# zhuhaozh/metadrive_ped

Hardware: AMD Instinct MI355X
Metric: agent-steps/sec at 4096 envs x 240-beam lidar (higher is better)
Workload: dtype f32; 1 GPU; BASELINE configs[1]: 4096 batched MetaDriveEnv per GPU, 3-block PG map (reference default block distribution: curves, straights, ramps, X/T intersections, roundabouts), 240-beam lidar, traffic_density=0.1, trigger traffic, auto-reset; envs_per_gpu=4096, agents_per_env=1, mover_capacity=24, n_beams=240

## Files before the change

### include/md_entity.h

```cpp
#ifndef MD_ENTITY_H
#define MD_ENTITY_H

#include "md_geom.h"
#include "md_lane_change.h"

MD_HD int md_scene_of_env(const MdState* g, int e) { return g->scene_of ? g->scene_of[e] : e; }
MD_HD size_t md_track_stride(const MdState* s, const MdConfig* c) {
    return (size_t)(s->walk.n_scenes > 0 ? s->walk.n_scenes : c->n_envs) * (size_t)c->cap;
}
MD_HD int md_scene(const MdState* s, int e) { return s->scene_of ? s->scene_of[0] : e; }

MD_HD MdState md_env_view(const MdState* g, const MdConfig* c, int e) {
    MdState v = *g;
    const size_t b = (size_t)e * (size_t)c->cap;
    const size_t bs = (size_t)md_scene_of_env(g, e) * (size_t)c->cap;
    const size_t a = (size_t)e * (size_t)c->agents_per_env;
    v.shape = g->shape + b;
    v.dyn = g->dyn ? g->dyn + b : 0;
    v.param = g->param ? g->param + b : 0;
    v.nav = g->nav ? g->nav + b : 0;
    v.pid = g->pid ? g->pid + b : 0;
    v.action = g->action ? g->action + 2 * b : 0;
    v.route_nodes = g->route_nodes ? g->route_nodes + b * MD_ROUTE_LEN : 0;
    v.route_roads = g->route_roads ? g->route_roads + b * MD_ROUTE_LEN : 0;
    v.final_lane = g->final_lane ? g->final_lane + b : 0;
    v.idm_rand = g->idm_rand ? g->idm_rand + b * MD_IDM_RAND : 0;
    v.flags = g->flags ? g->flags + b : 0;
    v.obs = g->obs ? g->obs + a * (size_t)c->obs_dim : 0;
    v.reward = g->reward ? g->reward + a : 0;
    v.cost = g->cost ? g->cost + a : 0;
    v.step_info = g->step_info ? g->step_info + a * 8 : 0;
    v.need_reset = g->need_reset ? g->need_reset + e : 0;
    v.shape0 = g->shape0 ? g->shape0 + b : 0;
    v.dyn0 = g->dyn0 ? g->dyn0 + b : 0;
    v.nav0 = g->nav0 ? g->nav0 + b : 0;
    v.pid0 = g->pid0 ? g->pid0 + b : 0;
    v.param0 = g->param0 ? g->param0 + b : 0;
    v.done_out = g->done_out ? g->done_out + 4 * a : 0;
    v.idle_ring = g->idle_ring ? g->idle_ring + a * MD_IDLE_WINDOW : 0;
    v.route_nodes0 = g->route_nodes0 ? g->route_nodes0 + b * MD_ROUTE_LEN : 0;
    v.route_roads0 = g->route_roads0 ? g->route_roads0 + b * MD_ROUTE_LEN : 0;
    v.final_lane0 = g->final_lane0 ? g->final_lane0 + b : 0;
    v.rng = g->rng ? g->rng + e : 0;
    v.env_steps = g->env_steps ? g->env_steps + e : 0;
    v.agent_id = g->agent_id ? g->agent_id + b : 0;
    v.next_agent_id = g->next_agent_id ? g->next_agent_id + e : 0;
    v.detected = g->detected ? g->detected + (size_t)e * c->agents_per_env * 2 : 0;
    v.agent_action = g->agent_action ? g->agent_action + (size_t)e * c->agents_per_env * 2 : 0;
    v.track_shape = g->track_shape ? g->track_shape + bs : 0;
    v.track_dyn = g->track_dyn ? g->track_dyn + 2 * bs : 0;
    v.scene_of = g->scene_of ? g->scene_of + e : 0;
    v.walk_ep = g->walk_ep ? g->walk_ep + e : 0;
    v.route_n = g->route_n ? g->route_n + 4 * b : 0;
    v.route_segs = g->route_segs ? g->route_segs + b * (size_t)c->route_seg_cap : 0;
    v.route_verts = g->route_verts ? g->route_verts + 2 * b * (size_t)c->route_vert_cap : 0;
    v.route_aux = g->route_aux ? g->route_aux + 8 * b : 0;
    return v;
}

MD_HD int md_obs_base(const MdConfig* c) { return c->random_agent_model ? 2 : 0; }
MD_HD int md_obs_mid(const MdConfig* c) { return md_obs_base(c) + (c->n_side > 0 ? c->n_side : 2); }
MD_HD int md_obs_ll(const MdConfig* c) { return md_obs_mid(c) + 6; }
MD_HD int md_obs_navi(const MdConfig* c) { return md_obs_ll(c) + (c->n_lane_line > 0 ? c->n_lane_line : 1); }
MD_HD int md_is_tollgate(const MdConfig* c) { return c->is_multi_agent && c->ma_kind == MD_MA_TOLLGATE; }
MD_HD int md_navi_dims(const MdConfig* c) { return md_is_tollgate(c) ? 0 : 10; }
MD_HD int md_obs_tail(const MdConfig* c) { return md_is_tollgate(c) ? 2 : 0; }
MD_HD int md_obs_others(const MdConfig* c) { return md_obs_navi(c) + md_navi_dims(c); }
MD_HD int md_others_width(const MdConfig* c) { return c->add_others_navi ? 8 : 4; }
MD_HD int md_obs_lidar(const MdConfig* c) { return md_obs_others(c) + (c->num_others > 0 ? c->num_others * md_others_width(c) : 0); }

MD_HD uint32_t md_done_word(uint32_t fl) {
    return ((fl & MD_FL_TERMINATED) ? 1u : 0u) | ((fl & MD_FL_TRUNCATED) ? 0x100u : 0u) | ((fl & 0xFFFFu) << 16);
}
MD_HD int md_kind_of(int flags) { return flags & MD_KIND_MASK; }
MD_HD int md_is_circle_kind(int k) { return k == MD_KIND_CONE || k == MD_KIND_WARNING || k == MD_KIND_PEDESTRIAN; }
MD_HD int md_present(int flags) { return (flags & MD_F_ALIVE) && md_kind_of(flags) != MD_KIND_NONE; }
MD_HD int md_drives(int flags) {
    return md_present(flags) && md_kind_of(flags) == MD_KIND_VEHICLE && !(flags & (MD_F_STATIC | MD_F_PENDING));
}

MD_HD int md_walks(int flags) {
    const int k = md_kind_of(flags);
    return (flags & MD_F_ALIVE) && !(flags & MD_F_STATIC) && (k == MD_KIND_PEDESTRIAN || k == MD_KIND_CYCLIST);
}
// ... 55 lines not shown
    float thr = md_sanitize(s->action[2 * n + 1]);
    s->action[2 * n] = steer;
    s->action[2 * n + 1] = thr;
    float yaw = (sh->s * d->last_c - sh->c * d->last_s) / (float)c->substeps;
    d->last_x = sh->cx;
    d->last_y = sh->cy;
    d->last_c = sh->c;
    d->last_s = sh->s;
    d->steering = steer;
    d->throttle = thr;
    float x = sh->cx, y = sh->cy, psi = d->heading, v = d->speed;
    MdBicycle bike;
    md_bicycle_prepare(steer, thr, v, sh->hl, sh->hw, c->dt, c->enable_reverse && (sh->flags & MD_F_AGENT), &s->param[n], &bike);
    float c0, s0;
    md_sincos(psi, &s0, &c0);
    float cp = c0 * bike.cb - s0 * bike.sb, sp = s0 * bike.cb + c0 * bike.sb;
    for (int k = 0; k < c->substeps; ++k) md_bicycle_substep(&x, &y, &psi, &v, &cp, &sp, &yaw, thr, &bike, &s->param[n], c->dt);
    sh->cx = x;
    sh->cy = y;
    d->heading = psi;
    d->speed = v;
    md_sincos(psi, &sh->s, &sh->c);
}


#define MD_OBS_TASKS 9

typedef struct MdObsCtx {
    const MdLane *lane, *ref0, *ref_last, *next0, *fin, *rl;
    float cur_w, cur_n, positive_road;
    int valid;
    int cur_block;
} MdObsCtx;

MD_HD void md_observe_ctx(const MdLane* lanes, const MdRoad* roads, const MdState* s, int n, MdObsCtx* k) {
    const MdShape* sh = &s->shape[n];
    const MdNav* nav = &s->nav[n];
    k->valid = md_drives(sh->flags) && nav->lane >= 0;
    k->lane = k->ref0 = k->ref_last = k->next0 = k->fin = k->rl = lanes;
    k->cur_w = k->cur_n = k->positive_road = 0.0f;
    k->cur_block = 0;
    if (!k->valid) return;
    const MdRoad* cur_road = &roads[nav->road0];
    k->cur_block = cur_road->block_kind;
    int has_next = nav->ck1 != nav->ck0;
    const MdRoad* next_road = has_next ? &roads[nav->road1] : cur_road;
    k->lane = &lanes[nav->lane];
    k->ref0 = &lanes[cur_road->first_lane];
    k->ref_last = &lanes[cur_road->first_lane + cur_road->n_lanes - 1];
    k->next0 = &lanes[next_road->first_lane];
    k->fin = &lanes[s->final_lane[n]];
    k->cur_w = k->lane->width;
    k->cur_n = (float)cur_road->n_lanes;
    k->positive_road = 1.0f;
    if (k->lane->road == nav->road0) k->rl = k->lane;
    else {
        k->rl = k->ref0;
        k->positive_road = cur_road->negative ? -1.0f : 1.0f;
    }
}

MD_HD void md_observe_task(int task, const MdObsCtx* k, const MdState* s, const MdConfig* c, int n, float* out5) {
    const MdShape* sh = &s->shape[n];
    const MdDyn* d = &s->dyn[n];
    float x = sh->cx, y = sh->cy;
    out5[0] = out5[1] = out5[2] = out5[3] = out5[4] = 0.0f;
    if (!k->valid) return;
    if (task == 0 || task == 2 || task == 5 || task == 6 || task == 7) {
        const MdLane* L = (task == 0) ? k->ref0 : ((task == 2) ? k->lane : ((task == 5) ? k->fin : k->rl));
        float px = (task == 6) ? d->last_x : x;
        float py = (task == 6) ? d->last_y : y;
        md_lane_local(L, px, py, &out5[0], &out5[1]);
    } else if (task == 3 || task == 4) {
        md_navi_for_checkpoint((task == 3) ? k->ref0 : k->next0, (k->cur_n / 2.0f - 0.5f) * k->cur_w, x, y, sh->c, sh->s,
                               k->cur_n, k->cur_w, c->curve_radius_max, c->curve_angle_max, out5);
    } else if (task == 1) {
        out5[0] = md_heading_diff(k->ref_last, x, y, sh->c, sh->s);
    } else if (task == 8) {
        float cosb = (sh->c * d->last_c + sh->s * d->last_s) / (md_norm(sh->c, sh->s) * md_norm(d->last_c, d->last_s));
        float beta = md_acos(md_clip(cosb, 0.0f, 1.0f));
        out5[0] = md_clip(beta / 0.1f, 0.0f, 1.0f);
        out5[1] = md_step_energy(md_fabs(d->speed) * 3.6f, md_norm(d->last_x - x, d->last_y - y));
    }
}

MD_HD void md_route_borders(const MdObsCtx* k, const float (*r)[5], float* to_left, float* to_right) {
    *to_left = r[0][1] + k->cur_w / 2.0f;
    *to_right = k->cur_w * k->cur_n - *to_left;
}

MD_HD void md_observe_state_dims(const MdObsCtx* k, const MdState* s, const MdConfig* c, int n, const float (*r)[5], float* obs) {
    const MdDyn* d = &s->dyn[n];
    const int o_mid = md_obs_mid(c), o_ll = md_obs_ll(c), o_navi = md_obs_navi(c);
    float to_left, to_right;
    md_route_borders(k, r, &to_left, &to_right);
    float speed_kmh = md_fabs(d->speed) * 3.6f;
    const MdParam* P = &s->param[n];
    const int o_base = md_obs_base(c);
    if (o_base) {
        obs[0] = md_clip(2.0f * s->shape[n].hl / 10.0f, 0.0f, 1.0f);
        obs[1] = md_clip(2.0f * s->shape[n].hw / 2.5f, 0.0f, 1.0f);
    }
    if (c->n_side <= 0) {
        obs[o_base + 0] = md_clip(to_left / c->total_width, 0.0f, 1.0f);
        obs[o_base + 1] = md_clip(to_right / c->total_width, 0.0f, 1.0f);
    }
    obs[o_mid + 0] = r[1][0];
    obs[o_mid + 1] = md_clip((speed_kmh + 1.0f) / (P->max_speed_kmh + 1.0f), 0.0f, 1.0f);
    obs[o_mid + 2] = md_clip((d->steering / 60.0f + 1.0f) / 2.0f, 0.0f, 1.0f);
    obs[o_mid + 3] = md_clip((s->action[2 * n] + 1.0f) / 2.0f, 0.0f, 1.0f);
    obs[o_mid + 4] = md_clip((s->action[2 * n + 1] + 1.0f) / 2.0f, 0.0f, 1.0f);
    obs[o_mid + 5] = r[8][0];
    float llat = r[2][1];
    if (c->n_lane_line <= 0) obs[o_ll] = md_clip((llat * 2.0f / c->max_lane_width + 1.0f) / 2.0f, 0.0f, 1.0f);
    if (!md_is_tollgate(c))
        for (int i = 0; i < 5; ++i) {
            obs[o_navi + i] = r[3][i];
            obs[o_navi + 5 + i] = r[4][i];
        }
}

MD_HD void md_observe_combine(const MdObsCtx* k, const MdState* s, const MdConfig* c, int a, int env_just_reset,
                              const float (*r)[5]) {
    int n = a;
    int just_reset = env_just_reset || ((s->shape[n].flags & MD_F_SPAWNED) != 0);
    s->shape[n].flags &= ~MD_F_SPAWNED;
    int ai = a;
    float* obs = s->obs + (size_t)ai * c->obs_dim;
    float* info = s->step_info + (size_t)ai * 8;
    MdDyn* d = &s->dyn[n];
    MdNav* nav = &s->nav[n];
    const int toll = md_is_tollgate(c);
    if (!k->valid) {
        if (s->done_out) ((uint32_t*)s->done_out)[ai] = 0u;
        for (int i = 0; i < md_obs_lidar(c); ++i) obs[i] = 0.0f;
        for (int i = c->obs_dim - md_obs_tail(c); i < c->obs_dim; ++i) obs[i] = 0.0f;
        s->reward[ai] = 0.0f;
        s->cost[ai] = 0.0f;
        for (int i = 0; i < 8; ++i) info[i] = 0.0f;
        return;
    }
    float cur_w = k->cur_w, cur_n = k->cur_n;

    float to_left, to_right;
    md_route_borders(k, r, &to_left, &to_right);
    uint32_t fl = s->flags[n] & (MD_FL_CRASH_VEHICLE | MD_FL_CRASH_OBJECT | MD_FL_CRASH_HUMAN | MD_FL_CRASH_BUILDING |
                                 MD_FL_CRASH_SIDEWALK | MD_FL_ON_WHITE_CONT | MD_FL_ON_YELLOW_CONT | MD_FL_ON_BROKEN |
                                 MD_FL_ON_CROSSWALK | MD_FL_ON_LANE);
    if (to_right < 0.0f || to_left < 0.0f) fl |= MD_FL_OUT_OF_ROUTE;

    md_observe_state_dims(k, s, c, n, r, obs);
    float speed_kmh = md_fabs(d->speed) * 3.6f;
    const MdParam* P = &s->param[n];
    float ls = r[2][0], llat = r[2][1];

    float fs = r[5][0], flat = r[5][1];
    int arrive = (k->fin->length - 5.0f < fs) && (fs < k->fin->length + 5.0f) && (cur_w / 2.0f >= flat) &&
                 (flat >= (0.5f - cur_n) * cur_w);
    int out_of_road = !(fl & MD_FL_ON_LANE);
    if (c->out_of_route_done) out_of_road = out_of_road || (fl & MD_FL_OUT_OF_ROUTE);
    else if (c->on_continuous_line_done)
        out_of_road = out_of_road || (fl & (MD_FL_ON_YELLOW_CONT | MD_FL_ON_WHITE_CONT | MD_FL_CRASH_SIDEWALK));
    if (toll) {
        out_of_road = (fl & MD_FL_CRASH_SIDEWALK) != 0;
        if (c->on_continuous_line_done) out_of_road = out_of_road || (fl & MD_FL_ON_YELLOW_CONT);
    }
// ... 767 lines not shown
```

### metadrive_ped_amd/csrc/mdstep.hip

```cpp
#include <hip/hip_runtime.h>
#include <stddef.h>
#include <stdint.h>
#include <stdio.h>
#include <stdlib.h>

#include <type_traits>

#include "md_curriculum.h"
#include "md_expert.h"
#include "md_expert_sense.h"
#include "md_ai_protect.h"
#include "md_scenario.h"
#include "md_topdown.h"
#include "md_render.h"

namespace {

constexpr int kBlock = 256;

enum Phase : int {
    PH_RESET = 1,
    PH_IDM = 2,
    PH_INTEGRATE = 4,
    PH_LOCALIZE = 8,
// ... 1307 lines not shown
template <bool kKeys>
__device__ __forceinline__ void idm_vehicle_wave(const MdWorld& w, const MdLane* lanes, const MdRoad* roads, const MdState& s,
                                 const MdConfig& c, int m, int slot, int lane_id, int* wave_list) {
    MdIdmPlan plan;
    plan.success = plan.use_ref = plan.fail = 0;
    plan.ids[0] = plan.ids[1] = plan.ids[2] = -1;
    const bool st_ = (slot == c.agents_per_env) && lane_id == 0;
    (void)st_;
    MD_FINE_STAMP(st_, 4);
    if (lane_id == 0) md_idm_plan(&w, lanes, roads, &s, &c, m, slot, &plan);
    if constexpr (!kKeys) {
        plan.success = bcast_i(plan.success, 0);
        plan.use_ref = bcast_i(plan.use_ref, 0);
        plan.fail = bcast_i(plan.fail, 0);
        plan.ids[0] = bcast_i(plan.ids[0], 0);
        plan.ids[1] = bcast_i(plan.ids[1], 0);
        plan.ids[2] = bcast_i(plan.ids[2], 0);
        MD_FINE_STAMP(st_, 5);
        FrontBack fb;
        idm_scan_wave(lanes, s, c, slot, lane_id, wave_list, plan, fb);
        MD_FINE_STAMP(st_, 6);
        if (lane_id == 0) md_idm_decide(lanes, roads, &s, slot, &plan, &fb);
    } else {
        plan.success = __builtin_amdgcn_readlane(plan.success, 0);
        plan.use_ref = __builtin_amdgcn_readlane(plan.use_ref, 0);
        plan.fail = __builtin_amdgcn_readlane(plan.fail, 0);
        plan.ids[0] = __builtin_amdgcn_readlane(plan.ids[0], 0);
        plan.ids[1] = __builtin_amdgcn_readlane(plan.ids[1], 0);
        plan.ids[2] = __builtin_amdgcn_readlane(plan.ids[2], 0);
        MD_FINE_STAMP(st_, 5);
        FrontBack fb;
        idm_scan_wave_keys(lanes, s, c, slot, lane_id, wave_list, plan, fb);
        MD_FINE_STAMP(st_, 6);
        if (lane_id == 0) {
            int front_obj;
            float front_dist;
            const float speed_kmh = md_fabs(s.dyn[slot].speed) * 3.6f;
            const int steer = md_idm_policy(lanes, roads, &s, slot, &plan, &fb, &front_obj, &front_dist);
            if (steer < 0) {
                s.action[2 * slot] = 0.0f;
                s.action[2 * slot + 1] = 0.0f;
            } else {
                const int k = (steer == plan.ids[0]) ? 0 : ((steer == plan.ids[1]) ? 1 : 2);
                const float* wf = reinterpret_cast<const float*>(wave_list);
                md_idm_act(&s, slot, speed_kmh, front_obj, front_dist, wf[kIdmLatWord + k], wf[kIdmHeadWord + k]);
            }
        }
    }
    MD_FINE_STAMP(st_, 7);
}

__device__ __forceinline__ void idm_group_wave(const MdWorld& w, const MdLane* lanes, const MdRoad* roads, const MdState& s,
                               const MdConfig& c, int m, int j0, unsigned long long mask, int lane_id, int* wave_list) {
    const int my_slot = j0 + lane_id;
    const bool mine = (mask >> lane_id) & 1ull;
    MdIdmPlan plan;
    plan.success = plan.use_ref = plan.fail = 0;
    plan.ids[0] = plan.ids[1] = plan.ids[2] = -1;
    if (mine) md_idm_plan(&w, lanes, roads, &s, &c, m, my_slot, &plan);
    FrontBack fb;
    front_back_clear(fb);
    unsigned long long todo = mask;
    while (todo) {
        const int v = __ffsll((long long)todo) - 1;
        todo &= todo - 1;
        MdIdmPlan up;
        up.success = bcast_i(plan.success, v);
        up.use_ref = bcast_i(plan.use_ref, v);
        up.fail = bcast_i(plan.fail, v);
        up.ids[0] = bcast_i(plan.ids[0], v);
        up.ids[1] = bcast_i(plan.ids[1], v);
        up.ids[2] = bcast_i(plan.ids[2], v);
        FrontBack ufb;
        idm_scan_wave(lanes, s, c, j0 + v, lane_id, wave_list, up, ufb);
        wave_lds_sync();
        if (lane_id == v) {
            plan.fail = up.fail;
            fb = ufb;
        }
    }
    if (mine) md_idm_decide(lanes, roads, &s, my_slot, &plan, &fb);
}

__device__ __forceinline__ void observe_agent_wave1(const MdLane* lanes, const MdRoad* roads, const MdState& s, const MdConfig& c, int a,
                                    int just_reset, int lane_id, float* wave_scratch ) {
    MdObsCtx k;
    MD_FINE_STAMP(a == 0 && lane_id == 0, 8);
    md_observe_ctx(lanes, roads, &s, a, &k);
    MD_FINE_STAMP(a == 0 && lane_id == 0, 9);
    if (lane_id < MD_OBS_TASKS) {
        float mine[5];
        md_observe_task(lane_id, &k, &s, &c, a, mine);
#pragma unroll
        for (int i = 0; i < 5; ++i) wave_scratch[lane_id * 5 + i] = mine[i];
    }
    wave_lds_sync();
    MD_FINE_STAMP(a == 0 && lane_id == 0, 10);
    if (lane_id == 0) md_observe_combine(&k, &s, &c, a, just_reset, (const float (*)[5])wave_scratch);
    __builtin_amdgcn_wave_barrier();
    MD_FINE_STAMP(a == 0 && lane_id == 0, 11);
}

constexpr int kObsGroups = 4;
constexpr int kObsScratch = kObsGroups * 48;

__device__ __forceinline__ void observe_agent_wave(const MdLane* lanes, const MdRoad* roads, const MdState& s, const MdConfig& c, int a_base,
                                   int just_reset, int lane_id, float* wave_scratch ) {
    const int g = lane_id >> 4, sub = lane_id & 15;
    const int a = a_base + g;
    const bool live = a < c.agents_per_env;
    float* scratch = wave_scratch + g * 48;
    MdObsCtx k;
    if (live) md_observe_ctx(lanes, roads, &s, a, &k);
    if (live && sub < MD_OBS_TASKS) {
        float mine[5];
        md_observe_task(sub, &k, &s, &c, a, mine);
#pragma unroll
        for (int i = 0; i < 5; ++i) scratch[sub * 5 + i] = mine[i];
    }
    wave_lds_sync();
    if (live && sub == 0) md_observe_combine(&k, &s, &c, a, just_reset, (const float (*)[5])scratch);
    __builtin_amdgcn_wave_barrier();
}

#ifndef MD_TRIGGER_EARLY
#define MD_TRIGGER_EARLY 1
#endif
constexpr int kNoTrigger = 0x7fffffff;
__device__ __forceinline__ void trigger_search_wave(const MdState& s, const MdConfig& c, int lane_id, int* min_order_out, int* trig_road_out) {
    const int base = 0;
    MD_FINE_STAMP(lane_id == 0, -1);
    *min_order_out = kNoTrigger;
    *trig_road_out = -1;
    int my_min = 0x7fffffff;
    for (int j = lane_id; j < c.cap; j += 64) {
        const int f = s.shape[base + j].flags;
        if ((f & MD_F_PENDING) && (f & MD_F_ALIVE)) {
            const int o = s.nav[base + j].trigger_order;
            my_min = o < my_min ? o : my_min;
        }
    }
    const int min_order = wave_min_i(my_min, my_min != 0x7fffffff, 0x7fffffff);
    if (min_order == 0x7fffffff) return;
    int my_slot = 0x7fffffff;
    for (int j = lane_id; j < c.cap; j += 64) {
        const int f = s.shape[base + j].flags;
        if ((f & MD_F_PENDING) && (f & MD_F_ALIVE) && s.nav[base + j].trigger_order == min_order)
            my_slot = j < my_slot ? j : my_slot;
    }
    const int first_slot = wave_min_i(my_slot, my_slot != 0x7fffffff, 0x7fffffff);
    *min_order_out = min_order;
    *trig_road_out = s.nav[base + first_slot].trigger_road;
    MD_FINE_STAMP(lane_id == 0, 14);
}

__device__ __forceinline__ void trigger_fire_wave(const MdLane* lanes, const MdState& s, const MdConfig& c, int lane_id, int min_order, int trig_road) {
    const int base = 0;
    if (min_order == kNoTrigger) return;
    bool fire = false;
    for (int a = lane_id; a < c.agents_per_env; a += 64) {
        if (!md_drives(s.shape[base + a].flags)) continue;
        const int al = s.nav[base + a].lane;
        if (al >= 0 && lanes[al].road == trig_road) fire = true;
    }
    if (__ballot(fire) == 0ull) return;
    for (int j = lane_id; j < c.cap; j += 64) {
        const int f = s.shape[base + j].flags;
        if ((f & MD_F_PENDING) && (f & MD_F_ALIVE) && s.nav[base + j].trigger_order == min_order)
            s.shape[base + j].flags = f & ~MD_F_PENDING;
    }
}

__device__ __forceinline__ void trigger_env(const MdLane* lanes, const MdState& s, const MdConfig& c, int lane_id) {
// ... 195 lines not shown
    s.param = img.param;
    s.final_lane = img.final_lane;
    return s;
}

struct SlotMask { unsigned long long lo, hi; };
static_assert(MD_MAX_CAP <= 128, "drive_mask: two 64-bit words per env");
__device__ __forceinline__ SlotMask drive_mask(const MdShape* shape, int cap, int lane) {
    SlotMask m = {0ull, 0ull};
    for (int j0 = 0; j0 < cap; j0 += 64) {
        const int j = j0 + lane;
        const unsigned long long mk = __ballot(j < cap && md_drives(shape[j < cap ? j : 0].flags));
        if (j0 == 0) m.lo = mk;
        else m.hi = mk;
    }
    return m;
}
__device__ __forceinline__ SlotMask agent_share(SlotMask m, int agents) {
    m.lo &= agents >= 64 ? ~0ull : ((1ull << agents) - 1ull);
    m.hi &= agents <= 64 ? 0ull : (agents >= 128 ? ~0ull : ((1ull << (agents - 64)) - 1ull));
    return m;
}
__device__ __forceinline__ int popc(SlotMask m) { return __popcll(m.lo) + __popcll(m.hi); }

#ifndef MD_ENV_BLOCK
#define MD_ENV_BLOCK 256
#endif
#ifndef MD_ENV_WAVES_EU
#define MD_ENV_WAVES_EU 7
#endif
template <class Config, class State, class Zero, class Null>
__host__ __device__ inline void lean_pins(Config& c, State& s, Zero zero, Null null) {
    zero(c.is_multi_agent);
    zero(c.traffic_mode);
    zero(c.agent_idm);
    zero(c.num_others);
    null(s.detected);
}
__host__ __device__ inline bool lean_pins_hold(const MdState& s, const MdConfig& c) {
    bool ok = true;
    lean_pins(c, s, [&ok](const int32_t& v) { ok = ok && v == 0; }, [&ok](const void* p) { ok = ok && p == nullptr; });
    return ok;
}
__host__ __device__ inline void lean_pins_fold(MdState& s, MdConfig& c) {
    lean_pins(c, s, [](int32_t& v) { v = 0; }, [](auto*& p) { p = nullptr; });
}

template <int PH, bool RESPAWN, bool MULTI>
constexpr int env_waves_per_eu() { return (PH == PH_ALL && !RESPAWN && !MULTI && MD_ENV_BLOCK >= 128) ? MD_ENV_WAVES_EU : 0; }

struct EnvLds { uint32_t shape, dyn, nav, pid, action, flags, lanes, roads, scratch, param, final_lane, det, onlane, cfl, tk, bytes; };
__host__ __device__ inline EnvLds env_lds(int cap, int agents, int n_lanes, int n_roads, int waves, bool multi, bool lidar_only) {
    EnvLds L;
    L.shape = 0;
    L.dyn = L.shape + (uint32_t)cap * sizeof(MdShape);
    L.nav = L.dyn + (uint32_t)cap * sizeof(MdDyn);
    L.pid = L.nav + (uint32_t)cap * sizeof(MdNav);
    L.action = L.pid + (uint32_t)cap * sizeof(MdPid);
    L.flags = L.action + (uint32_t)cap * 2 * sizeof(float);
    L.lanes = align_up(L.flags + (uint32_t)cap * sizeof(uint32_t), 16);
    L.roads = L.lanes + (uint32_t)n_lanes * sizeof(MdLane);
    L.scratch = L.roads + (uint32_t)n_roads * sizeof(MdRoad);
    L.param = L.scratch + (uint32_t)waves * (multi ? kObsScratch : 48) * sizeof(float);
    L.final_lane = L.param + (uint32_t)cap * sizeof(MdParam);
    L.det = L.final_lane + align_up(cap, 2) * sizeof(int32_t);
    L.onlane = L.det + (uint32_t)agents * 2 * sizeof(unsigned long long);
    L.cfl = L.onlane + (uint32_t)cap * sizeof(uint32_t);
    const uint32_t shared_words = 2 * cap > 8 ? 2 * cap : 8;
    L.tk = L.onlane + shared_words * sizeof(uint32_t);
    L.bytes = lidar_only ? L.dyn : L.tk + 3 * sizeof(int);
    return L;
}

template <int PH, bool STAGE_MAP, bool RESPAWN = false, bool MULTI = false, int BLK = MD_ENV_BLOCK>
__global__ __launch_bounds__(BLK)
__attribute__((amdgpu_waves_per_eu(env_waves_per_eu<PH, RESPAWN, MULTI>() ? env_waves_per_eu<PH, RESPAWN, MULTI>() : 1,
                                   env_waves_per_eu<PH, RESPAWN, MULTI>() ? env_waves_per_eu<PH, RESPAWN, MULTI>() : 8)))
void env_kernel(MdWorld w, MdState g, MdConfig c, float* lidar_out,
                                                  int lidar_stride, int lidar_offset) {
    constexpr int kBlock = BLK;
    constexpr int kWaves = kBlock / 64;
    constexpr bool kIdmKeys = !STAGE_MAP && !RESPAWN && !MULTI;
    constexpr bool kLocRoadFirst = PH == PH_ALL ? kIdmKeys : PH == PH_LOCALIZE_ROAD_FIRST;
    if constexpr (PH == PH_ALL && !RESPAWN && !MULTI && !STAGE_MAP) lean_pins_fold(g, c);
    if ((int)blockIdx.x >= c.n_envs) return;
#ifdef MD_STAMP
    const int e = g_env_order ? g_env_order[blockIdx.x] : (int)blockIdx.x;
#else
    const int e = blockIdx.x;
#endif
    const int tid = threadIdx.x;
    const int wave = tid >> 6, lane = tid & 63;
    const int cap = c.cap;

    const int n_stage_lanes = STAGE_MAP ? w.max_lanes : 0, n_stage_roads = STAGE_MAP ? w.max_roads : 0;
    constexpr bool kLidarOnly = (PH == PH_LIDAR);
    const EnvLds L = env_lds(cap, c.agents_per_env, n_stage_lanes, n_stage_roads, kWaves, MULTI, kLidarOnly);
    extern __shared__ __attribute__((aligned(16))) unsigned char smem[];
    MdShape* l_shape = reinterpret_cast<MdShape*>(smem + L.shape);
    MdDyn* l_dyn = reinterpret_cast<MdDyn*>(smem + L.dyn);
    MdNav* l_nav = reinterpret_cast<MdNav*>(smem + L.nav);
    MdPid* l_pid = reinterpret_cast<MdPid*>(smem + L.pid);
    float* l_action = reinterpret_cast<float*>(smem + L.action);
    uint32_t* l_flags = reinterpret_cast<uint32_t*>(smem + L.flags);
    MdLane* l_lanes = reinterpret_cast<MdLane*>(smem + L.lanes);
    MdRoad* l_roads = reinterpret_cast<MdRoad*>(smem + L.roads);
    float* l_scratch = reinterpret_cast<float*>(smem + L.scratch) + wave * (MULTI ? kObsScratch : 48);
    MdParam* l_param = reinterpret_cast<MdParam*>(smem + L.param);
    int32_t* l_final = reinterpret_cast<int32_t*>(smem + L.final_lane);
    unsigned long long* l_det = reinterpret_cast<unsigned long long*>(smem + L.det);
    const EnvImage img = {l_shape, l_dyn, l_pid, l_param, l_nav, l_action, l_flags, l_final};
    uint32_t* l_onlane = reinterpret_cast<uint32_t*>(smem + L.onlane);
    uint32_t* l_cfl = reinterpret_cast<uint32_t*>(smem + L.cfl);
    int* l_tk = reinterpret_cast<int*>(smem + L.tk);
    const bool track_det = (PH == PH_ALL) && (RESPAWN || MULTI) && g.detected != nullptr;

    const MdState gv = md_env_view(&g, &c, e);
    const int reset_flag = (PH & PH_RESET) ? gv.need_reset[0] : 0;

    MD_STAMP_AT(0);
    const bool kFusedAct = (PH == PH_ALL) && gv.agent_action != nullptr;
    const MdLane* lanes;
    const MdRoad* roads;
    if (STAGE_MAP) {
        lanes = l_lanes;
        roads = l_roads;
    } else {
        lanes = w.lanes + w.lane_off[w.env_map[e]];
        roads = w.roads + w.road_off[w.env_map[e]];
    }
    if (kLidarOnly) {
        copy16(l_shape, gv.shape, cap * (int)sizeof(MdShape), tid, kBlock);
    } else if (kBlock >= 256) {
        const int n32 = cap * 2, n64 = cap * 4;
        const uint4* g_shape = reinterpret_cast<const uint4*>(gv.shape);
        const uint4* g_dyn = reinterpret_cast<const uint4*>(gv.dyn);
        const uint4* g_pid = reinterpret_cast<const uint4*>(gv.pid);
        const uint4* g_param = reinterpret_cast<const uint4*>(gv.param);
        const uint4* g_nav = reinterpret_cast<const uint4*>(gv.nav);
        uint4 r_shape, r_dyn, r_pid, r_param, r_nav0;
        float2 r_act;
        uint32_t r_fl;
        int r_fin;
        const bool p32 = tid < n32, pc = tid < cap;
        if (p32) {
            r_shape = ld_stream(&g_shape[tid]);
            r_dyn = ld_stream(&g_dyn[tid]);
            r_pid = ld_stream(&g_pid[tid]);
            r_param = ld_stream(&g_param[tid]);
        }
        if (tid < n64) r_nav0 = ld_stream(&g_nav[tid]);
        if (pc) {
            r_act = (kFusedAct && tid < c.agents_per_env) ? reinterpret_cast<const float2*>(gv.agent_action)[tid]
                                                          : reinterpret_cast<const float2*>(gv.action)[tid];
            r_fl = gv.flags[tid];
            r_fin = gv.final_lane ? gv.final_lane[tid] : 0;
        }
        if (STAGE_MAP) {
            const int m = w.env_map[e];
            const int lo = w.lane_off[m], ro = w.road_off[m];
            copy16(l_lanes, w.lanes + lo, (w.lane_off[m + 1] - lo) * (int)sizeof(MdLane), tid, kBlock);
            copy16(l_roads, w.roads + ro, (w.road_off[m + 1] - ro) * (int)sizeof(MdRoad), tid, kBlock);
        }
        if (p32) {
            reinterpret_cast<uint4*>(l_shape)[tid] = r_shape;
            reinterpret_cast<uint4*>(l_dyn)[tid] = r_dyn;
// ... 111 lines not shown
            }
            if (RESPAWN) md_advance_mover(&s, &c, j);
            else md_integrate_mover(&s, &c, j);
        }
        if (!RESPAWN)
            for (int j = tid; j < cap; j += kBlock) md_walk_mover(&s, &c, j);
        __syncthreads();
    }
    MD_STAMP_AT(4);
    unsigned long long drv_lo = 0ull, drv_hi = 0ull;
    if (kFused) {
        const SlotMask drv = drive_mask(s.shape, cap, lane);
        drv_lo = drv.lo;
        drv_hi = drv.hi;
        const SlotMask adrv = agent_share(drv, c.agents_per_env);
        const unsigned long long adrv_lo = adrv.lo, adrv_hi = adrv.hi;
        const int nd = popc(drv), na = popc(adrv);
        if (MULTI) {
            const int npair = (nd + 1) >> 1;
            for (int guard = 0; guard < npair + na; ++guard) {
                int item = 0;
                if (lane == 0) item = atomicAdd(&l_tk[0], 1);
                item = __builtin_amdgcn_readfirstlane(item);
                if (item < 0 || item >= npair + na) break;
                if (item < na) contacts_vehicle(w, s, c, e, kth_bit(adrv_lo, adrv_hi, item), lane, l_cfl);
                else localize_pair(w, lanes, roads, s, e, kth_bit(drv_lo, drv_hi, 2 * (item - na)), kth_bit(drv_lo, drv_hi, 2 * (item - na) + 1), lane, l_onlane);
            }
        } else if (nd + na <= kWaves) {
            for (int item = wave; item < nd + na; item += kWaves) {
                if (item < nd) {
                    if (!(MD_ENV_SKIP & 4)) localize_vehicle<kLocRoadFirst>(w, lanes, roads, s, e, kth_bit(drv_lo, drv_hi, item), lane, l_onlane);
                } else if (!(MD_ENV_SKIP & 8)) contacts_vehicle(w, s, c, e, kth_bit(adrv_lo, adrv_hi, item - nd), lane, l_cfl);
            }
        } else {
            const int npair = (nd + 1) >> 1;
            for (int item = wave; item < npair + na; item += kWaves) {
                if (item < npair) {
                    if (!(MD_ENV_SKIP & 4)) localize_pair<kLocRoadFirst>(w, lanes, roads, s, e, kth_bit(drv_lo, drv_hi, 2 * item), kth_bit(drv_lo, drv_hi, 2 * item + 1), lane, l_onlane);
                } else if (!(MD_ENV_SKIP & 8))
                    contacts_vehicle(w, s, c, e, kth_bit(adrv_lo, adrv_hi, item - npair), lane, l_cfl);
            }
        }
        __syncthreads();
    } else {
        if (PH & PH_LOCALIZE) {
            for (int j = wave; j < cap; j += kWaves) localize_vehicle<kLocRoadFirst>(w, lanes, roads, s, e, j, lane);
            __syncthreads();
        }
        MD_STAMP_AT(5);
        if (PH & PH_CONTACTS) {
            for (int j = wave; j < cap; j += kWaves) contacts_vehicle(w, s, c, e, j, lane);
            __syncthreads();
        }
    }
    MD_STAMP_AT(6);
    if (PH & PH_TRAFFIC) {
        for (int j = tid; j < cap; j += kBlock) {
            const bool drove = kFused ? ((((j < 64) ? (drv_lo >> j) : (drv_hi >> (j - 64))) & 1ull) != 0ull) : false;
            if (kFused && !drove) continue;
            const int f = s.shape[j].flags;
            if (kFused)
                s.flags[j] = l_onlane[j] | ((f & MD_F_AGENT) ? l_cfl[j] : 0u);
            if (md_drives(f) && !(f & MD_F_AGENT) && !(s.flags[j] & MD_FL_ON_LANE)) {
                s.shape[j].flags = f & ~MD_F_ALIVE;
                if (kFused) l_cfl[j] = kRemovedMark;
            }
        }
        if (plan_ahead && wave == kWaves - 1) {
            if (kTriggerEarly) {
                const int* l_trig = reinterpret_cast<const int*>(smem + L.scratch) + kTrigWord;
                trigger_fire_wave(lanes, s, c, lane, __builtin_amdgcn_readfirstlane(l_trig[0]), __builtin_amdgcn_readfirstlane(l_trig[1]));
            } else trigger_env(lanes, s, c, lane);
        }
        __syncthreads();
        if (RESPAWN) {
            if (tid == 0) md_traffic_respawn_env(&w, lanes, &s, &c, w.env_map[e]);
            __syncthreads();
        }
    }
    MD_STAMP_AT(7);
    if (plan_ahead) {
        if (wave == 0) {
            if (!(MD_ENV_SKIP & 16))
                for (int a = 0; a < c.agents_per_env; ++a) observe_agent_wave1(lanes, roads, s, c, a, just_reset, lane, l_scratch);
        } else if (!(MD_ENV_SKIP & 2)) {
            int rank = 0;
            for (int j0 = 0; j0 < cap; j0 += 64) {
                const int jl = j0 + lane;
                const int fl = (jl < cap) ? s.shape[jl].flags : 0;
                unsigned long long mk = __ballot(jl < cap && md_drives(fl) && !(fl & MD_F_AGENT));
                while (mk) {
                    const int j = j0 + __ffsll((long long)mk) - 1;
                    mk &= mk - 1;
                    if (rank % (kWaves - 1) == wave - 1) idm_vehicle_wave<kIdmKeys>(w, lanes, roads, s, c, w.env_map[e], j, lane, reinterpret_cast<int*>(l_scratch));
                    ++rank;
                }
            }
        }
        MD_STAMP_AT(8);
    } else if (PH & PH_OBSERVE) {
        if (MULTI) {
            const int n_grp = (c.agents_per_env + kObsGroups - 1) / kObsGroups;
            for (int guard = 0; guard < n_grp; ++guard) {
                int gi = 0;
                if (lane == 0) gi = atomicAdd(&l_tk[1], 1);
                gi = __builtin_amdgcn_readfirstlane(gi);
                if (gi < 0 || gi >= n_grp) break;
                observe_agent_wave(lanes, roads, s, c, gi * kObsGroups, just_reset, lane, l_scratch);
            }
        } else {
            for (int a = wave; a < c.agents_per_env; a += kWaves) observe_agent_wave1(lanes, roads, s, c, a, just_reset, lane, l_scratch);
        }
        MD_STAMP_AT(8);
    }
    if ((PH & PH_LIDAR) && !(PH == PH_ALL && (MD_ENV_SKIP & 1))) {
        if (c.n_beams > 0) phase_lidar(w, s, c, e, tid, kWaves, lidar_out, lidar_stride, lidar_offset, track_det ? l_det : nullptr, PH == PH_ALL ? &l_tk[2] : nullptr);
    }

    MD_STAMP_AT(9);
    if (!kLidarOnly) {
        __syncthreads();
        MD_STAMP_AT(10);
        constexpr bool respawns = (PH & PH_TRAFFIC) && RESPAWN;
        if (kFused && !MULTI && !do_reset) {
            const bool replay = c.traffic_mode == 3;
            auto dirty = [&](int j) { return replay || md_moves(l_shape[j].flags) || l_cfl[j] == kRemovedMark; };
            for (int i = tid; i < cap * 2; i += kBlock)
                if (dirty(i >> 1)) {
                    st_stream(&reinterpret_cast<uint4*>(gv.shape)[i], reinterpret_cast<const uint4*>(l_shape)[i]);
                    st_stream(&reinterpret_cast<uint4*>(gv.dyn)[i], reinterpret_cast<const uint4*>(l_dyn)[i]);
                    st_stream(&reinterpret_cast<uint4*>(gv.pid)[i], reinterpret_cast<const uint4*>(l_pid)[i]);
                }
            for (int i = tid; i < cap * 4; i += kBlock)
                if (dirty(i >> 2)) st_stream(&reinterpret_cast<uint4*>(gv.nav)[i], reinterpret_cast<const uint4*>(l_nav)[i]);
            for (int j = tid; j < cap; j += kBlock)
                if (dirty(j)) {
                    reinterpret_cast<float2*>(gv.action)[j] = reinterpret_cast<const float2*>(l_action)[j];
                    gv.flags[j] = l_flags[j];
                    if (RESPAWN) gv.final_lane[j] = l_final[j];
                }
            if (track_det)
                for (int j = tid; j < 2 * c.agents_per_env; j += kBlock) gv.detected[j] = l_det[j];
            MD_STAMP_AT(11);
            return;
        }
        if (PH & (PH_RESET | PH_IDM | PH_INTEGRATE | PH_TRAFFIC | PH_OBSERVE | PH_LIFECYCLE)) copy16(gv.shape, l_shape, cap * (int)sizeof(MdShape), tid, kBlock);
        if (MULTI && (PH & (PH_RESET | PH_LIFECYCLE)) && c.random_agent_model && c.is_multi_agent)
            copy16(gv.param, l_param, cap * (int)sizeof(MdParam), tid, kBlock);
        if ((PH & (PH_RESET | PH_INTEGRATE | PH_LIFECYCLE)) || respawns) copy16(gv.dyn, l_dyn, cap * (int)sizeof(MdDyn), tid, kBlock);
        if ((PH & (PH_RESET | PH_IDM | PH_LOCALIZE | PH_OBSERVE | PH_LIFECYCLE)) || respawns) copy16(gv.nav, l_nav, cap * (int)sizeof(MdNav), tid, kBlock);
        if ((PH & (PH_RESET | PH_IDM | PH_OBSERVE | PH_LIFECYCLE)) || respawns || (lane_change && (PH & PH_INTEGRATE)))
            copy16(gv.pid, l_pid, cap * (int)sizeof(MdPid), tid, kBlock);
        if (((PH & (PH_RESET | PH_LIFECYCLE)) && MULTI) || ((PH & (PH_RESET | PH_TRAFFIC)) && RESPAWN)) {
            for (int j = tid; j < cap; j += kBlock) gv.final_lane[j] = l_final[j];
        }
        for (int j = tid; j < cap; j += kBlock) {
            if ((PH & (PH_RESET | PH_IDM | PH_INTEGRATE | PH_LIFECYCLE)) || respawns) {
                gv.action[2 * j] = l_action[2 * j];
                gv.action[2 * j + 1] = l_action[2 * j + 1];
            }
            if ((PH & (PH_RESET | PH_LOCALIZE | PH_CONTACTS | PH_OBSERVE | PH_LIFECYCLE)) || respawns) gv.flags[j] = l_flags[j];
        }
        if (track_det)
            for (int j = tid; j < 2 * c.agents_per_env; j += kBlock) gv.detected[j] = l_det[j];
        if (do_reset && tid == 0) gv.need_reset[0] = 0;
    }
    MD_STAMP_AT(11);
// ... 2831 lines not shown
```

Measured before the change: 58.54 million agent-steps/s.

## Compute observation tasks in lockstep across 16 lanes with branch-free selects

Replaces the per-lane divergent observation task dispatch with a single branch-free routine in which 16 wave lanes each compute one output. Lanes choose their lane pointer, field offsets and formula operands through mask-based selects, and inline reduced atan/asin polynomials replace the library calls. The aim is to remove SIMD divergence, since the different task branches (lane-local, navigation checkpoints, heading, energy) would otherwise serialize within the wave. The cost is duplicated arithmetic on every lane, plus inline asm and polynomial approximations that may differ slightly in numerics.

```diff
diff --git a/include/md_entity.h b/include/md_entity.h
--- a/include/md_entity.h
+++ b/include/md_entity.h
@@ -1,5 +1,7 @@
 #ifndef MD_ENTITY_H
 #define MD_ENTITY_H
+
+#include <stddef.h>
 
 #include "md_geom.h"
 #include "md_lane_change.h"
@@ -221,6 +223,170 @@
         out5[0] = md_clip(beta / 0.1f, 0.0f, 1.0f);
         out5[1] = md_step_energy(md_fabs(d->speed) * 3.6f, md_norm(d->last_x - x, d->last_y - y));
     }
+}
+
+#define MD_OBS_LANES 16
+#if defined(__HIP_DEVICE_COMPILE__)
+#define MD_LANE_IN(lane, mask) __extension__({ unsigned long long m_; __asm__ volatile("s_mov_b64 %0, %1" : "=s"(m_) : "i"(mask)); __builtin_amdgcn_inverse_ballot_w64(m_); })
+#else
+#define MD_LANE_IN(lane, mask) ((((mask) >> (lane)) & 1ull) != 0)
+#endif
+#define MD_LANE_F(m) ((int)(offsetof(MdLane, m) / sizeof(float)))
+
+MD_HD float md_atan_reduced(float xr, float y0, int neg) {
+    float z = xr * xr;
+    y0 += (((8.05374449538e-2f * z - 1.38776856032e-1f) * z + 1.99777106478e-1f) * z - 3.33329491539e-1f) * z * xr + xr;
+    return neg ? -y0 : y0;
+}
+
+MD_HD float md_asin_small(float x) {
+    float z = x * x;
+    return ((((4.2163199048e-2f * z + 2.4181311049e-2f) * z + 4.5470025998e-2f) * z + 7.4953002686e-2f) * z
+            + 1.6666752422e-1f) * z * x + x;
+}
+
+MD_HD void md_observe_lane(int lane, const MdObsCtx* k, const MdState* s, const MdConfig* c, int n, float* r45) {
+    if (!k->valid) return;
+    const MdShape* sh = &s->shape[n];
+    const MdDyn* d = &s->dyn[n];
+    const float x = sh->cx, y = sh->cy, hc = sh->c, hs = sh->s;
+    const float last_x = d->last_x, last_y = d->last_y, last_c = d->last_c, last_s = d->last_s, speed = d->speed;
+    const int task = (lane < 9) ? lane : ((lane == 9) ? 8 : 3 + (lane & 1));
+#define MD_LF 0x00E5ull
+#define MD_LN 0x0C18ull
+#define MD_LH 0x0002ull
+#define MD_LY 0x0100ull
+#define MD_LE 0x0200ull
+#define MD_LB 0x3000ull
+#define MD_LA 0xC000ull
+#define MD_PICK(m, v, e) do { const int p_ = MD_LANE_IN(lane, m); v = p_ ? (e) : v; } while (0)
+#define MD_PICK2(m, v, e, w, f) do { const int p_ = MD_LANE_IN(lane, m); v = p_ ? (e) : v; w = p_ ? (f) : w; } while (0)
+    const char* const ref0 = (const char*)k->ref0;
+    int o_rec = 0;
+    MD_PICK(0x0002ull, o_rec, (int)((const char*)k->ref_last - ref0));
+    MD_PICK(0x0004ull, o_rec, (int)((const char*)k->lane - ref0));
+    MD_PICK(0xA810ull, o_rec, (int)((const char*)k->next0 - ref0));
+    MD_PICK(0x0020ull, o_rec, (int)((const char*)k->fin - ref0));
+    MD_PICK(0x00C0ull, o_rec, (int)((const char*)k->rl - ref0));
+    const MdLane* L = (const MdLane*)(ref0 + o_rec);
+    const float* lf = (const float*)L;
+    int i0 = MD_LANE_F(ax), i1 = MD_LANE_F(ay), i2 = MD_LANE_F(bx), i3 = MD_LANE_F(by);
+    int i4 = MD_LANE_F(end_phase_w), i5 = MD_LANE_F(end_phase);
+    MD_PICK2(MD_LN, i0, MD_LANE_F(ex), i1, MD_LANE_F(ey));
+    MD_PICK2(MD_LN, i2, MD_LANE_F(elx), i3, MD_LANE_F(ely));
+    MD_PICK2(MD_LH, i2, MD_LANE_F(ex), i3, MD_LANE_F(ey));
+    MD_PICK2(MD_LH, i4, MD_LANE_F(sx), i5, MD_LANE_F(sy));
+    MD_PICK(MD_LA, i2, MD_LANE_F(angle));
+    const float g0 = lf[i0], g1 = lf[i1], g2 = lf[i2], g3 = lf[i3], g4 = lf[i4], g5 = lf[i5];
+    const float g6 = L->dirsign, g7 = L->length;
+    const int type = L->type;
+
+    float px = x, py = y;
+    MD_PICK2(0x0040ull, px, last_x, py, last_y);
+    const float later_middle = (k->cur_n / 2.0f - 0.5f) * k->cur_w;
+    const float fa = px - g0, fb = py - g1;
+    const int h_straight = (int)MD_LANE_IN(lane, MD_LH) & (type == 0);
+    float a = 1.0f, b = 0.0f;
+    MD_PICK2(MD_LF, a, fa, b, fb);
+    MD_PICK2(MD_LN, a, (g0 + later_middle * g2) - x, b, (g1 + later_middle * g3) - y);
+    MD_PICK2(MD_LH, a, h_straight ? g2 - g4 : ((g6 > 0.0f) ? fa : g0 - x), b, h_straight ? g3 - g5 : ((g6 > 0.0f) ? fb : g1 - y));
+    MD_PICK2(MD_LY, a, hc, b, hs);
+    MD_PICK2(MD_LE, a, last_x - x, b, last_y - y);
+
+    const float n1 = md_norm(a, b);
+    float a2 = 1.0f, b2 = 0.0f;
+    MD_PICK2(MD_LY, a2, last_c, b2, last_s);
+    MD_PICK2(MD_LH, a2, hc, b2, hs);
+    const float n2 = md_norm(a2, b2);
+
+    const int curved = type == 1;
+    float num1 = 0.0f, den1 = 1.0f;
+    MD_PICK2(MD_LF, num1, fb, den1, fa);
+    MD_PICK2(MD_LN, num1, a, den1, n1);
+    MD_PICK2(MD_LH, num1, b, den1, n1);
+    MD_PICK2(MD_LY, num1, hc * last_c + hs * last_s, den1, n1 * n2);
+    MD_PICK2(MD_LE, num1, n1, den1, 1000.0f);
+    MD_PICK2(MD_LB, num1, g2, den1, c->curve_radius_max + k->cur_n * k->cur_w);
+    MD_PICK2(MD_LA, num1, (curved ? g2 : 0.0f) * 57.29577951308232f, den1, c->curve_angle_max);
+    float out1 = ((curved ? -g6 : 0.0f) + 1.0f) / 2.0f;
+    const float q1 = num1 / den1;
+    float out0 = (q1 + 1.0f) / 2.0f;
+    MD_PICK(MD_LB, out0, (type == 1) ? q1 : 0.0f);
+
+    const int at_neg = q1 < 0.0f;
+    const float at_x = at_neg ? -q1 : q1;
+    const int at_big = at_x > 2.414213562373095f, at_mid = !at_big && at_x > 0.4142135623730950f;
+    const float at_y0 = at_big ? MD_HALF_PI_F : (at_mid ? MD_QUARTER_PI_F : 0.0f);
+    float num2 = 0.0f, den2 = 1.0f;
+    MD_PICK2(MD_LF, num2, at_big ? -1.0f : (at_mid ? at_x - 1.0f : at_x), den2, at_big ? at_x : (at_mid ? at_x + 1.0f : 1.0f));
+    MD_PICK2(MD_LN, num2, b, den2, n1);
+    MD_PICK2(MD_LH, num2, -a, den2, n1);
+    const float q2 = num2 / den2;
+
+    if (MD_LANE_IN(lane, MD_LF)) {
+        out0 = fa * g2 + fb * g3;
+        out1 = fa * g3 - fb * g2;
+        if (type != 0) {
+            float abs_phase = md_atan_reduced(q2, at_y0, q1 < 0.0f);
+            abs_phase = (fa < 0.0f) ? ((fb < 0.0f) ? abs_phase - MD_PI_F : abs_phase + MD_PI_F) : abs_phase;
+            abs_phase = (fb == 0.0f) ? ((fa > 0.0f) ? 0.0f : MD_PI_F) : abs_phase;
+            abs_phase = (fa == 0.0f) ? ((fb > 0.0f) ? MD_HALF_PI_F : ((fb < 0.0f) ? -MD_HALF_PI_F : 0.0f)) : abs_phase;
+            const float radius = g2, start_phase = g3;
+            const float d_start = md_fabs(md_wrap_to_pi(abs_phase - start_phase));
+            const float d_end = md_fabs(md_wrap_to_pi(abs_phase - g4));
+            const int clockwise = g6 < 0.0f, from_end = d_start > d_end;
+            const float phase0 = from_end ? g5 : start_phase;
+            const float along = md_wrap_to_pi(clockwise ? (phase0 - abs_phase) : (abs_phase - phase0)) * radius;
+            out0 = from_end ? along + g7 : along;
+            out1 = g6 * (n1 - radius);
+        }
+    }
+
+    const float NAVI_POINT_DIST = 50.0f;
+    const int cut = (int)MD_LANE_IN(lane, MD_LN) & (n1 > NAVI_POINT_DIST);
+    const int h_quot = (int)MD_LANE_IN(lane, MD_LH) & (type == 0);
+    const float vx = cut ? q1 * NAVI_POINT_DIST : (h_quot ? q1 : a);
+    const float vy = cut ? q2 * NAVI_POINT_DIST : (h_quot ? q2 : b);
+
+    const float cosb = md_clip(q1, 0.0f, 1.0f);
+    const int ac_hi = (int)MD_LANE_IN(lane, MD_LY) & (cosb > 0.5f);
+    const float n3 = md_sqrt(h_quot ? vx * vx + vy * vy : (ac_hi ? 0.5f * (1.0f - cosb) : 1.0f));
+    const float ln = h_quot ? n3 : n1;
+
+    float num3 = vx * hc + vy * hs, den3 = NAVI_POINT_DIST;
+    MD_PICK(0x0C00ull, num3, vy * hc - vx * hs);
+    MD_PICK2(MD_LH, num3, hc * vx + hs * vy, den3, ln * n2);
+    if (MD_LANE_IN(lane, MD_LY)) {
+        num3 = ac_hi ? 2.0f * md_asin_small(n3) : MD_HALF_PI_F - md_asin_small(cosb);
+        den3 = 0.1f;
+    }
+    if (MD_LANE_IN(lane, MD_LE)) {
+        float t = 3.25f * md_exp(0.01f * (md_fabs(speed) * 3.6f));
+        num3 = t * q1;
+        den3 = 100.0f;
+    }
+    const float q3 = num3 / den3;
+
+    int w0 = task * 5;
+    MD_PICK2(MD_LN, out0, (q3 + 1.0f) / 2.0f, w0, w0 + (lane >= 10));
+    MD_PICK(MD_LH, out0, (!(ln * n2 != 0.0f)) ? 0.0f : md_clip(q3, -1.0f, 1.0f) / 2.0f + 0.5f);
+    MD_PICK(MD_LY, out0, q3);
+    MD_PICK2(MD_LE, out0, q3 * 1000.0f, w0, w0 + 1);
+    MD_PICK(MD_LB, w0, w0 + 2);
+    MD_PICK(MD_LA, w0, w0 + 4);
+
+    MD_PICK(0xFD18ull, out0, md_clip(out0, 0.0f, 1.0f));
+    if (MD_LANE_IN(lane, 0xFFFFull)) r45[w0] = out0;
+    if (MD_LANE_IN(lane, MD_LF | MD_LB)) r45[w0 + 1] = (lane >= 12) ? md_clip(out1, 0.0f, 1.0f) : out1;
+#undef MD_PICK
+#undef MD_PICK2
+#undef MD_LF
+#undef MD_LN
+#undef MD_LH
+#undef MD_LY
+#undef MD_LE
+#undef MD_LB
+#undef MD_LA
 }
 
 MD_HD void md_route_borders(const MdObsCtx* k, const float (*r)[5], float* to_left, float* to_right) {
diff --git a/metadrive_ped_amd/csrc/mdstep.hip b/metadrive_ped_amd/csrc/mdstep.hip
--- a/metadrive_ped_amd/csrc/mdstep.hip
+++ b/metadrive_ped_amd/csrc/mdstep.hip
@@ -1413,13 +1413,20 @@
     if (mine) md_idm_decide(lanes, roads, &s, my_slot, &plan, &fb);
 }
 
+#ifndef MD_OBS_LOCKSTEP
+#define MD_OBS_LOCKSTEP 1
+#endif
+template <bool kLockstep = false>
 __device__ __forceinline__ void observe_agent_wave1(const MdLane* lanes, const MdRoad* roads, const MdState& s, const MdConfig& c, int a,
                                     int just_reset, int lane_id, float* wave_scratch ) {
     MdObsCtx k;
     MD_FINE_STAMP(a == 0 && lane_id == 0, 8);
     md_observe_ctx(lanes, roads, &s, a, &k);
     MD_FINE_STAMP(a == 0 && lane_id == 0, 9);
-    if (lane_id < MD_OBS_TASKS) {
+    if constexpr (kLockstep) {
+        if (lane_id < MD_OBS_TASKS * 5) wave_scratch[lane_id] = 0.0f;
+        md_observe_lane(lane_id, &k, &s, &c, a, wave_scratch);
+    } else if (lane_id < MD_OBS_TASKS) {
         float mine[5];
         md_observe_task(lane_id, &k, &s, &c, a, mine);
 #pragma unroll
@@ -1781,6 +1788,7 @@
     constexpr int kWaves = kBlock / 64;
     constexpr bool kIdmKeys = !STAGE_MAP && !RESPAWN && !MULTI;
     constexpr bool kLocRoadFirst = PH == PH_ALL ? kIdmKeys : PH == PH_LOCALIZE_ROAD_FIRST;
+    constexpr bool kObsLockstep = MD_OBS_LOCKSTEP && PH == PH_ALL && kIdmKeys;
     if constexpr (PH == PH_ALL && !RESPAWN && !MULTI && !STAGE_MAP) lean_pins_fold(g, c);
     if ((int)blockIdx.x >= c.n_envs) return;
 #ifdef MD_STAMP
@@ -2058,7 +2066,7 @@
     if (plan_ahead) {
         if (wave == 0) {
             if (!(MD_ENV_SKIP & 16))
-                for (int a = 0; a < c.agents_per_env; ++a) observe_agent_wave1(lanes, roads, s, c, a, just_reset, lane, l_scratch);
+                for (int a = 0; a < c.agents_per_env; ++a) observe_agent_wave1<kObsLockstep>(lanes, roads, s, c, a, just_reset, lane, l_scratch);
         } else if (!(MD_ENV_SKIP & 2)) {
             int rank = 0;
             for (int j0 = 0; j0 < cap; j0 += 64) {
```

Measured after the change: 59.59 million agent-steps/s, median of 6. +1.8%, better.
